# ConsenSys/wittgenstein

Hardware: NVIDIA H100
Metric: simulated-ms/sec, GSFSignature 65,536 nodes (higher is better)
Workload: dtype u64 bitmaps / int32

## Files before the change

### wittgenstein_b200/csrc/wtg_cuda.cu

```cuda
#include <cuda_runtime.h>
#include <unistd.h>

#include <cstdio>
#include <cstdlib>
#include <stdexcept>
#include <string>
#include <vector>

#include "wtg_engine.hpp"

namespace wtg {

#define CUDA_OK(x)                                                                                       \
  do {                                                                                                   \
    cudaError_t e_ = (x);                                                                                \
    if (e_ != cudaSuccess) throw std::runtime_error(std::string("CUDA: ") + cudaGetErrorString(e_) + " at " #x); \
  } while (0)

constexpr int SCAN_THREADS = 256;
constexpr int SCAN_ITEMS = 4;
constexpr int SCAN_TILE = SCAN_THREADS * SCAN_ITEMS;

__global__ void k_begin(Dev d, int mode) {
  if (threadIdx.x >= 32) return;
// ... 97 lines not shown
    for (int n = d.n0; n < d.n0 + d.nLoc; ++n) idx += (u64)hCondPick(d, n, idx, true);
  }
}
__global__ void k_hpick_publish(Dev d) {
  const int blk = blockIdx.x, nBlk = gridDim.x;
  if (!d.ctl->error)
    for (int n = d.n0 + blk * blockDim.x + threadIdx.x; n < d.n0 + d.nLoc; n += nBlk * blockDim.x) hPickPublish(d, n);
  if (blk == 0 && threadIdx.x == 0) hPickPublishHeader(d);
}
__global__ void k_hpick_xcheck(Dev d) {
  if (d.ctl->error) return;
  const int blk = blockIdx.x, nBlk = gridDim.x;
  if (blk == 0 && threadIdx.x == 0) hPickHeaders(d);
  const int upTo = hPicksBelow(d, d.rank + 1);
  for (int t = blk * blockDim.x + threadIdx.x; t < upTo; t += nBlk * blockDim.x)
    if (hPickRejects(d, t)) d.ctl->hReject = 1;
}
__global__ void k_hpick_xapply(Dev d) {
  if (d.ctl->error) return;
  const int blk = blockIdx.x, nBlk = gridDim.x;
  if (!d.ctl->hReject) {
    const u64 below = (u64)hPicksBelow(d, d.rank);
    for (int n = d.n0 + blk * blockDim.x + threadIdx.x; n < d.n0 + d.nLoc; n += nBlk * blockDim.x) hCondPick(d, n, below + (u64)d.hDrawBase[n], true);
  } else if (blk == 0 && threadIdx.x == 0) {
    hPickSerial(d);
  }
}

__global__ void k_dispatch_count(Dev d) {
  if (d.ctl->error) return;
  const int blk = blockIdx.x, nBlk = gridDim.x;
  int nEv = d.ctl->nEv;
  if (d.allCap > 0) {
    CoopWarp c;
    int gw = (blk * blockDim.x + threadIdx.x) >> 5, nw = (nBlk * blockDim.x) >> 5;
    for (int i = gw; i < nEv; i += nw) dispatchCountCoop(d, c, i);
    return;
  }
  for (int i = blk * blockDim.x + threadIdx.x; i < nEv; i += nBlk * blockDim.x) dispatchCount(d, i);
}
__global__ void k_dispatch_scatter(Dev d) {
  if (d.ctl->error) return;
  const int blk = blockIdx.x, nBlk = gridDim.x;
  int nEv = d.ctl->nEv;
  if (d.allCap > 0) {
    CoopWarp c;
    int gw = (blk * blockDim.x + threadIdx.x) >> 5, nw = (nBlk * blockDim.x) >> 5;
    for (int i = gw; i < nEv; i += nw) dispatchScatterCoop(d, c, i);
    return;
  }
  for (int i = blk * blockDim.x + threadIdx.x; i < nEv; i += nBlk * blockDim.x) dispatchScatter(d, i);
}

__global__ void __launch_bounds__(256) k_node_msgs(Dev d) {
  if (d.ctl->error) return;
  const int blk = blockIdx.x;
  int n = d.n0 + blk * blockDim.x + threadIdx.x;
  int flag = 0;
  u64 word = ~0ULL;
  if (n < d.n0 + d.nLoc && d.inboxFill[n] > 0) {
    CoopSerial cs;
    if (d.proto == PROTO_SANFERMIN || d.proto == PROTO_CAPPOS || d.proto == PROTO_SLUSH || d.proto == PROTO_SNOWFLAKE ||
        d.proto == PROTO_P2PFLOOD)
      nodeProcess(d, cs, n, 0);
    else if (d.proto == PROTO_GSF || d.proto == PROTO_PINGPONG) {
      u64 w = 0;
      int tasks = nodeProcess(d, cs, n, 1, &w);
      flag = tasks > 0 ? 1 : 0;
      if (tasks == 1) word = w;
    }
    else if (d.proto == PROTO_CASPER) {
      const u64* in = d.inbox + d.inboxOff[n];
      const Ev* bucket = d.buckets + (size_t)(d.ctl->tick & (d.ring - 1)) * (size_t)d.bcap;
      int cnt = d.inboxFill[n];
      bool simple = true;
      for (int r = 0; r < cnt && simple; ++r) {
        const Ev& ev = bucket[inboxEntry(in[r])];
        uint32_t meta = ev.kind == EV_MULTI ? d.rec[ev.aux].meta : ev.meta;
        simple = (ev.kind == EV_MSG || ev.kind == EV_MULTI) && meta == CM_ATT;
      }
      if (simple)
        nodeProcess(d, cs, n, 0);
      else
        flag = 1;
    } else
      flag = 1;
  }
  listAppend(d, flag != 0, n, d.ctl->taskCnt, d.taskList, d.taskWord, word);
}
__global__ void __launch_bounds__(256, 3) k_node_tasks(Dev d) {
  if (d.ctl->error) return;
  const int blk = blockIdx.x, nBlk = gridDim.x;
  const bool split = d.proto == PROTO_GSF || d.proto == PROTO_PINGPONG;
  const int stripe = blk & (ARENA_STRIPES - 1);
  const int cnt = d.ctl->taskCnt[stripe];
  const int sub = (blk >> 6) * 8 + (threadIdx.x >> 5);
  const int nsub = (nBlk >> 6) * 8;
  const int* list = d.taskList + (size_t)stripe * d.listStripeCap;
  const u64* words = d.taskWord + (size_t)stripe * d.listStripeCap;
  CoopWarp c;
  for (int t = sub; t < cnt; t += nsub) {
    const int n = list[t];
    const u64 w = words[t];
    if (split && w != ~0ULL)
      nodeSingleTask(d, c, n, w);
    else
      nodeProcess(d, c, n, split ? 2 : 0);
  }
}
__global__ void k_casper_fixups(Dev d) {
  const int blk = blockIdx.x;
  if (d.ctl->error || blk != 0 || threadIdx.x >= 32) return;
  CoopWarp c;
  if (d.cRandomTies && d.ctl->tieCnt > 0) casperResolveTies(d, c);
  if (d.G == 1 && d.cg->createdThisTick > 1) casperRenumber(d, c);
}
__device__ __forceinline__ Pair pairAdd(Pair x, Pair y) {
  Pair r;
  r.a = x.a + y.a;
  r.b = x.b + y.b;
  return r;
}
__device__ __forceinline__ Pair blockExclusive(Pair v, Pair& total) {
  __shared__ Pair warpSums[33];
  int lane = threadIdx.x & 31, warp = threadIdx.x >> 5, nw = blockDim.x >> 5;
  Pair inc = v;
#pragma unroll
  for (int o = 1; o < 32; o <<= 1) {
    int ta = __shfl_up_sync(0xffffffffu, inc.a, o), tb = __shfl_up_sync(0xffffffffu, inc.b, o);
    if (lane >= o) {
      inc.a += ta;
      inc.b += tb;
    }
  }
  __syncthreads();
  if (lane == 31) warpSums[warp] = inc;
  __syncthreads();
  if (warp == 0) {
    Pair w;
    w.a = lane < nw ? warpSums[lane].a : 0;
    w.b = lane < nw ? warpSums[lane].b : 0;
    Pair wi = w;
#pragma unroll
    for (int o = 1; o < 32; o <<= 1) {
      int ta = __shfl_up_sync(0xffffffffu, wi.a, o), tb = __shfl_up_sync(0xffffffffu, wi.b, o);
      if (lane >= o) {
        wi.a += ta;
        wi.b += tb;
      }
    }
    Pair ex;
    ex.a = wi.a - w.a;
    ex.b = wi.b - w.b;
    warpSums[lane] = ex;
    if (lane == 31) warpSums[32] = wi;
  }
  __syncthreads();
  total = warpSums[32];
  Pair base = warpSums[warp];
  Pair r;
// ... 292 lines not shown
        if (d.G > 1) d.newTarget[g] = -1;
      }
      __syncwarp();
    }
    __syncthreads();
  }
}

__global__ void k_free(Dev d) {
  if (d.ctl->error) return;
  const int blk = blockIdx.x, nBlk = gridDim.x;
  const int per = d.freeCap / ARENA_STRIPES;
  const int stripe = blk & (ARENA_STRIPES - 1);
  int cnt = d.ctl->freeCnt[stripe];
  if (cnt > per) cnt = per;
  const int sub = (blk >> 6) * blockDim.x + threadIdx.x;
  const int nsub = (nBlk >> 6) * blockDim.x;
  for (int j = sub; j < cnt; j += nsub) freeApply(d, stripe * per + j);
}

__global__ void k_gsf_init_nodes(Dev d) {
  int n = d.n0 + blockIdx.x * blockDim.x + threadIdx.x;
  if (n < d.n0 + d.nLoc) gsfInitNodeBody(d, n);
}
__global__ void k_rng_candidates(Dev d, u64 s0, u64 count, u64 chunk, int maxBound, u64* out, int* outCount, int cap) {
  u64 t = (u64)blockIdx.x * blockDim.x + threadIdx.x;
  u64 start = t * chunk;
  if (start >= count) return;
  u64 len = start + chunk <= count ? chunk : count - start;
  rngCandidateChunk(d, s0, start, len, maxBound, out, outCount, cap);
}
template <class PeerT>
__global__ void k_gsf_shuffle(Dev d, int l, u64 s0, const int* liveRank, const u64* rejOrd, int nRej) {
  int n = d.n0 + blockIdx.x * blockDim.x + threadIdx.x;
  if (n < d.n0 + d.nLoc) gsfShuffleLevel<PeerT>(d, n, l, s0, liveRank, rejOrd, nRej);
}

class CudaBackend : public Backend {
 public:
  cudaStream_t st = nullptr;
  cudaStream_t side = nullptr;
  cudaEvent_t forkEv = nullptr, joinEv = nullptr;
  int devId = 0;
  void bind() const { cudaSetDevice(devId); }
  int sms = 132;
  int smemOptin = 0;
  cudaGraphExec_t tickGraph = nullptr;
  const void* graphFor = nullptr;
  bool useGraph = true;
  long long launches = 0;
  long long graphKernels = 0;
  cudaEvent_t tm0 = nullptr, tm1 = nullptr;
  enum ProfSlot { P_BEGIN, P_COND_SCAN, P_DISPATCH_COUNT, P_SCAN_PARTIAL, P_EXCHANGE, P_SCAN_FINAL, P_DISPATCH_SCATTER, P_NODE,
                  P_EMIT, P_MS_COUNT, P_MS_SCAN, P_MS_SCATTER, P_FREE, P_END, P_COND_SCORE, P_COND_SELECT, P_EMIT_PEERS, NK };
  bool profiling = false;
  std::vector<cudaEvent_t> evPool;
  std::vector<int> evKernel;
  size_t evUsed = 0;
  double profMs[NK] = {};
  long long profCnt[NK] = {};
  const char* profNames[NK] = {"k_begin", "k_cond_scan", "k_dispatch_count", "k_scan_partial", "k_exchange", "k_scan_final",
                               "k_dispatch_scatter", "k_node", "k_emit", "k_ms_count", "k_ms_scan", "k_ms_scatter", "k_free",
                               "k_end", "k_cond_score", "k_cond_select", "k_emit_peers"};

  explicit CudaBackend(int requested = -1) {
    int dev = 0;
    const char* e = std::getenv("LOCAL_RANK");
    int cnt = 0;
    CUDA_OK(cudaGetDeviceCount(&cnt));
    if (cnt == 0) throw std::runtime_error("no CUDA device");
    if (e) dev = std::atoi(e) % cnt;
    const char* e2 = std::getenv("WTG_DEVICE");
    if (e2) dev = std::atoi(e2) % cnt;
    if (requested >= 0) {
      if (requested >= cnt) throw std::invalid_argument("CUDA device " + std::to_string(requested) + " does not exist");
      dev = requested;
    }
    CUDA_OK(cudaSetDevice(dev));
    devId = dev;
    cudaDeviceProp p;
    CUDA_OK(cudaGetDeviceProperties(&p, dev));
    sms = p.multiProcessorCount;
    CUDA_OK(cudaStreamCreateWithFlags(&st, cudaStreamNonBlocking));
    CUDA_OK(cudaStreamCreateWithFlags(&side, cudaStreamNonBlocking));
    CUDA_OK(cudaEventCreateWithFlags(&forkEv, cudaEventDisableTiming));
    CUDA_OK(cudaEventCreateWithFlags(&joinEv, cudaEventDisableTiming));
    CUDA_OK(cudaDeviceGetAttribute(&smemOptin, cudaDevAttrMaxSharedMemoryPerBlockOptin, dev));
    CUDA_OK(cudaFuncSetAttribute(k_ms_count, cudaFuncAttributeMaxDynamicSharedMemorySize, smemOptin));
    CUDA_OK(cudaFuncSetAttribute(k_ms_scatter, cudaFuncAttributeMaxDynamicSharedMemorySize, smemOptin));
    const char* g = std::getenv("WTG_NO_GRAPH");
    if (g && g[0] == '1') useGraph = false;
  }
  ~CudaBackend() override {
    for (void* q : ipcOpened) cudaIpcCloseMemHandle(q);
    if (tickGraph) cudaGraphExecDestroy(tickGraph);
    if (forkEv) cudaEventDestroy(forkEv);
    if (joinEv) cudaEventDestroy(joinEv);
    if (side) cudaStreamDestroy(side);
    if (st) cudaStreamDestroy(st);
  }
  void* alloc(size_t bytes) override {
    bind();
    void* p = nullptr;
    cudaError_t e = cudaMalloc(&p, bytes);
    if (e != cudaSuccess) throw std::runtime_error("cudaMalloc of " + std::to_string(bytes) + " bytes failed: " + cudaGetErrorString(e));
    CUDA_OK(cudaMemsetAsync(p, 0, bytes, st));
    return p;
  }
  void release(void* p) override { cudaFree(p); }
  int deviceId() const override { return devId; }
  void exportShared(void* p, unsigned char* handle) override {
    bind();
    std::memset(handle, 0, 128);
    cudaIpcMemHandle_t ih;
    CUDA_OK(cudaIpcGetMemHandle(&ih, p));
    static_assert(sizeof(ih) == 64, "cudaIpcMemHandle_t");
// ... 11 lines not shown
    int dev;
    std::memcpy(&pid, handle + 64, 8);
    std::memcpy(&p, handle + 72, sizeof(p));
    std::memcpy(&dev, handle + 80, 4);
    if (pid == (long long)getpid()) {
      if (dev != devId) {
        int can = 0;
        CUDA_OK(cudaDeviceCanAccessPeer(&can, devId, dev));
        if (!can) throw std::runtime_error("GPU " + std::to_string(devId) + " cannot access GPU " + std::to_string(dev) + " (peer access)");
        cudaError_t e = cudaDeviceEnablePeerAccess(dev, 0);
        if (e != cudaSuccess && e != cudaErrorPeerAccessAlreadyEnabled) CUDA_OK(e);
        cudaGetLastError();
      }
      return p;
    }
    cudaIpcMemHandle_t ih;
    std::memcpy(&ih, handle, 64);
    void* q = nullptr;
    CUDA_OK(cudaIpcOpenMemHandle(&q, ih, cudaIpcMemLazyEnablePeerAccess));
    ipcOpened.push_back(q);
    return q;
  }
  void upload(void* dst, const void* src, size_t bytes) override {
    bind();
    CUDA_OK(cudaMemcpyAsync(dst, src, bytes, cudaMemcpyHostToDevice, st));
    CUDA_OK(cudaStreamSynchronize(st));
  }
  void download(void* dst, const void* src, size_t bytes) override {
    bind();
    CUDA_OK(cudaMemcpyAsync(dst, src, bytes, cudaMemcpyDeviceToHost, st));
    CUDA_OK(cudaStreamSynchronize(st));
  }
  void sync() override {
    bind();
    CUDA_OK(cudaStreamSynchronize(st));
    drainProfile();
  }
  void timerStart() override {
    bind();
    if (!tm0) {
      CUDA_OK(cudaEventCreate(&tm0));
      CUDA_OK(cudaEventCreate(&tm1));
    }
    CUDA_OK(cudaEventRecord(tm0, st));
  }
  double timerStopMs() override {
    bind();
    CUDA_OK(cudaEventRecord(tm1, st));
    CUDA_OK(cudaEventSynchronize(tm1));
    float ms = 0;
    CUDA_OK(cudaEventElapsedTime(&ms, tm0, tm1));
    return (double)ms;
  }
  void profileEnable(bool on) override {
    sync();
    profiling = on;
    if (on) {
      for (int i = 0; i < NK; ++i) {
        profMs[i] = 0;
        profCnt[i] = 0;
      }
    }
  }
  int profileRead(double* ms, long long* cnt, const char** names, int cap) override {
    sync();
    int k = 0;
    for (int i = 0; i < NK && k < cap; ++i, ++k) {
      ms[k] = profMs[i];
      cnt[k] = profCnt[i];
      names[k] = profNames[i];
    }
    return k;
  }
  void drainProfile() {
    for (size_t i = 0; i < evUsed; ++i) {
      float ms = 0;
      cudaEventElapsedTime(&ms, evPool[2 * i], evPool[2 * i + 1]);
      profMs[evKernel[i]] += ms;
      profCnt[evKernel[i]] += 1;
    }
    evUsed = 0;
  }
  void profBegin(int kid) {
    if (!profiling) return;
    if (evUsed * 2 + 2 > evPool.size()) {
      if (evUsed >= 8192) {
        CUDA_OK(cudaStreamSynchronize(st));
        drainProfile();
      } else {
        cudaEvent_t a, b;
        CUDA_OK(cudaEventCreate(&a));
        CUDA_OK(cudaEventCreate(&b));
        evPool.push_back(a);
        evPool.push_back(b);
        evKernel.push_back(0);
      }
    }
    evKernel[evUsed] = kid;
    CUDA_OK(cudaEventRecord(evPool[2 * evUsed], st));
  }
  void profEnd() {
    if (!profiling) return;
    CUDA_OK(cudaEventRecord(evPool[2 * evUsed + 1], st));
    ++evUsed;
  }

  void fork() {
    CUDA_OK(cudaEventRecord(forkEv, st));
    CUDA_OK(cudaStreamWaitEvent(side, forkEv, 0));
  }
  void join() {
    CUDA_OK(cudaEventRecord(joinEv, side));
    CUDA_OK(cudaStreamWaitEvent(st, joinEv, 0));
  }
  void enqueueTick(const Dev& d, int mode) {
    const int wide = sms * 8;
    const size_t msSmem = (size_t)d.msWarps * d.ring * sizeof(int);
    const bool branches = mode == 1 && !profiling && d.G == 1 && (d.proto == PROTO_GSF || d.proto == PROTO_HANDEL);
    cudaStream_t sd = branches ? side : st;
    if (mode != 3) {
      profBegin(P_BEGIN);
      k_begin<<<1, 32, 0, st>>>(d, mode);
      profEnd();
// ... 4 lines not shown
      profBegin(P_COND_SCAN);
      k_cond_mark<<<(d.nLoc + 255) / 256, 256, 0, st>>>(d);
      k_cond_nodes<0><<<ARENA_STRIPES * 19, 256, 0, st>>>(d);
      profEnd();
      profBegin(P_COND_SCORE);
      k_cond_score<<<ARENA_STRIPES * 19, 256, 0, st>>>(d);
      profEnd();
      profBegin(P_COND_SELECT);
      k_cond_nodes<1><<<ARENA_STRIPES * 19, 256, smem8, st>>>(d);
      profEnd();
      launches += 4;
      if (d.proto == PROTO_HANDEL) {
        Dev dd = d;
        dd.scanPartial = d.drawScanPartial;
        profBegin(P_SCAN_PARTIAL);
        k_scan_partial<<<wide, SCAN_THREADS, 0, st>>>(dd, 2);
        profEnd();
        profBegin(P_SCAN_FINAL);
        k_scan_final<<<wide, SCAN_THREADS, 0, st>>>(dd, 2);
        profEnd();
        if (d.G > 1) {
          profBegin(P_EXCHANGE);
          k_hpick_publish<<<sms, 256, 0, st>>>(d);
          k_x_sync<<<1, 32, 0, st>>>(d, 3);
          profEnd();
          profBegin(P_COND_SELECT);
          k_hpick_xcheck<<<sms, 256, 0, st>>>(d);
          k_hpick_xapply<<<sms, 256, 0, st>>>(d);
          profEnd();
          launches += 5;
        } else {
          profBegin(P_COND_SELECT);
          k_hpick_check<<<sms, 256, 0, st>>>(d);
          k_hpick_apply<<<sms, 256, 0, st>>>(d);
          profEnd();
          launches += 3;
        }
      }
    }
    if (mode != 2 && mode != 3) {
      profBegin(P_DISPATCH_COUNT);
      k_dispatch_count<<<wide, 256, 0, sd>>>(d);
      profEnd();
      profBegin(P_SCAN_PARTIAL);
      k_scan_partial<<<wide, SCAN_THREADS, 0, sd>>>(d, 0);
      profEnd();
      profBegin(P_SCAN_FINAL);
      k_scan_final<<<wide, SCAN_THREADS, 0, sd>>>(d, 0);
      profEnd();
      profBegin(P_DISPATCH_SCATTER);
      k_dispatch_scatter<<<wide, 256, 0, sd>>>(d);
      profEnd();
      if (branches) join();
      profBegin(P_NODE);
      k_node_msgs<<<(d.nLoc + 255) / 256, 256, 0, st>>>(d);
      k_node_tasks<<<ARENA_STRIPES * 19, 256, 0, st>>>(d);
      if (d.proto == PROTO_CASPER) {
        k_casper_fixups<<<1, 32, 0, st>>>(d);
        launches += 1;
      }
      profEnd();
      launches += 6;
    }
    profBegin(P_SCAN_PARTIAL);
    k_scan_partial<<<wide, SCAN_THREADS, 0, st>>>(d, 1);
    profEnd();
    profBegin(P_SCAN_FINAL);
    k_scan_final<<<wide, SCAN_THREADS, 0, st>>>(d, 1);
    profEnd();
    if (d.G > 1) {
      profBegin(P_EXCHANGE);
      k_x1_publish<<<sms * 2, 256, 0, st>>>(d);
      k_x_sync<<<1, 32, 0, st>>>(d, 0);
      k_x1_totals<<<1, 1, 0, st>>>(d);
      k_x1_offsets<<<sms * 2, 256, 0, st>>>(d);
      profEnd();
      launches += 4;
    }
    profBegin(P_EMIT);
    if (d.shufCap > 0) {
      k_shuffle_check<<<ARENA_STRIPES * 4, 256, 0, st>>>(d);
      k_shuffle_serial<<<1, 1, 0, st>>>(d);
      launches += 2;
    }
    k_emit<<<ARENA_STRIPES * 16, 256, 0, st>>>(d);
    if (d.allCap > 0) {
      if (d.G > 1)
        k_x_all_publish<<<8, 128, 0, st>>>(d);
      else
        k_emit_all<<<d.allWarps / 4, 128, 0, st>>>(d);
      launches += 1;
    }
    profEnd();
    if (d.proto == PROTO_P2PFLOOD) {
      profBegin(P_EMIT_PEERS);
      k_emit_peers<<<sms * 8, 128, 0, st>>>(d);
      profEnd();
      launches += 1;
    }
    if (d.G > 1) {
      profBegin(P_EXCHANGE);
      k_x_sync<<<1, 32, 0, st>>>(d, 1);
      k_x2_ingest<<<sms * 4, 256, 0, st>>>(d);
      launches += 2;
      if (d.allCap > 0) {
        k_x_all_build<<<d.allWarps / 4, 128, 0, st>>>(d);
        launches += 1;
      }
      profEnd();
// ... 111 lines not shown
```

### wittgenstein_b200/csrc/wtg_engine.hpp

```cpp
#pragma once
#include <chrono>
#include <cstdio>
#include <functional>
#include <thread>
#include <cstdlib>
#include <cstring>
#include <memory>
#include <string>
#include <vector>

#include "wtg_host.hpp"
#include "wtg_logic.cuh"
#include "wtg_types.h"

namespace wtg {

struct GsfParams {
  int nodeCount, threshold, pairingTime, timeoutPerLevelMs, periodDurationMs, acceleratedCallsCount, nodesDown;
};

struct SfParams {
  int nodeCount, threshold, pairingTime, signatureSize, replyTimeout, candidateCount;
};

struct HandelParams {
  int nodeCount, threshold, pairingTime, levelWaitTime, extraCycle, disseminationPeriodMs, fastPath, nodesDown, desynchronizedStart,
      byzantineSuicide, hiddenByzantine;
};

struct CapposParams {
  int nodeCount, threshold, pairingTime, signatureSize, timeout, candidateCount;
};

struct CasperParams {
  int cycleLength, randomOnTies, blockProducersCount, attestersPerRound, blockConstructionTime, attestationConstructionTime;
};

struct Tunables {
  long long bcap = 0, qcap = 0, poolSlotsPerNode = 0, descCap = 0, recCap = 0, ring = 0;
  long long casperVotes = 0;
  long long casperBlocks = 0;
  long long peerBits32 = 0;
  long long farCap = 0;
  long long stageWords = 0;
};

struct Backend {
  virtual ~Backend() {}
  virtual void* alloc(size_t bytes) = 0;
  virtual void release(void* p) = 0;
  virtual void upload(void* dst, const void* src, size_t bytes) = 0;
  virtual void download(void* dst, const void* src, size_t bytes) = 0;
  virtual void sync() = 0;
  virtual void tick(const Dev& d, int mode) = 0;
  virtual void ticks(const Dev& d, int count) {
    for (int i = 0; i < count; ++i) tick(d, 1);
  }
  virtual void timerStart() {}
  virtual double timerStopMs() { return 0.0; }
  virtual void profileEnable(bool) {}
  virtual int profileRead(double* ms, long long* launches, const char** names, int cap) { (void)ms; (void)launches; (void)names; (void)cap; return 0; }
  virtual void* allocShared(size_t bytes) { return alloc(bytes); }
  virtual void exportShared(void* p, unsigned char* handle) {
    std::memset(handle, 0, 128);
    std::memcpy(handle + 72, &p, sizeof(p));
  }
  virtual void* importShared(const unsigned char* handle) {
    void* p;
    std::memcpy(&p, handle + 72, sizeof(p));
    return p;
  }
  virtual int deviceId() const { return 0; }
  virtual void gsfInitNodes(const Dev& d) = 0;
  virtual void rngCandidates(const Dev& d, unsigned long long s0, unsigned long long count, int maxBound,
                             std::vector<unsigned long long>& out) = 0;
  virtual void gsfShufflePeers(const Dev& d, unsigned long long s0, const int* liveRank, const unsigned long long* rejOrd, int nRej) = 0;
};

class Engine {
 public:
  std::unique_ptr<Backend> be;
  HostModel hm;
  Dev d;
  Tunables tun;
  std::vector<void*> allocs;
  bool inited = false;
  int time = 0;
  int ringMask = 0;
  bool pendingAtNow = false;
  std::vector<int> partitionsInX;
  int msgDiscardTime = 0x7fffffff;
  std::string err;
  std::vector<int> liveRank;
  unsigned long long initDraws = 0;

  int shardRank = 0, shardWorld = 1;
  bool linked = false;
  void* xRegion = nullptr;
  size_t xBytes = 0;
  long long stageWordsWanted = 0;
  long long farWanted = 0;
  struct XLayout {
    size_t hdr, flags, items, newEv, newTarget, stage, rec, recDest, recArrival, beg, all, allCnt, proto, total;
  } xl{};
  size_t xProtoBytes = 0;
  int xAllCapWanted = 0;
  bool unevenShards = false;
  bool shardFarOk = false;

  explicit Engine(Backend* b) : be(b) { std::memset(&d, 0, sizeof(d)); }
  void setShard(int rank, int world) {
    requireNotInited();
    if (world < 1 || world > MAX_SHARDS || (world & (world - 1)) != 0) throw std::invalid_argument("the number of shards must be a power of two <= 8");
// ... 1756 lines not shown
```

### wittgenstein_b200/csrc/wtg_logic.cuh

```cuda
#pragma once
#include "wtg_types.h"

template <class T, class U>
static inline T wtg_host_fetch_add(T* p, U v) {
  T o = *p;
  *p = (T)(o + (T)v);
  return o;
}
template <class T>
static inline T wtg_host_fetch_max(T* p, T v) {
  T o = *p;
  if (v > o) *p = v;
  return o;
}
template <class T>
static inline T wtg_host_fetch_min(T* p, T v) {
  T o = *p;
  if (v < o) *p = v;
  return o;
}
template <class T>
static inline T wtg_host_cas(T* p, T a, T b) {
  T o = *p;
  if (o == a) *p = b;
// ... 650 lines not shown
  return st * per + i;
}

WTG_HD void gsfLevelCounters(const Dev& d, int n, int l, int& cV, int& cI, int& cU) {
  cV = d.cntVer[n * d.L + l];
  cI = d.cntIndiv[n * d.L + l];
  cU = d.cntUnion[n * d.L + l];
}


template <class C>
WTG_HD int gsfLastFinishedLevel(const Dev& d, C& c, int n) {
  uint32_t comp = 0;
  for (int k = 0; k < 32 / C::LANES; ++k) {
    const int l = k * C::LANES + c.lane();
    comp |= c.ballot(l >= 1 && l < d.L && d.cntVer[n * d.L + l] == (1 << (l - 1))) << (k * C::LANES);
  }
  return WTG_CTZ32(~(comp >> 1));
}

WTG_HD void gsfOnNewSig(const Dev& d, int n, uint32_t from, uint32_t meta, u64 pl) {
  int l = (int)metaLevel(meta);
  int len = d.qLen[n];
  QEntry* q = d.queue + (size_t)n * d.qcap;
  if (len + 2 > d.qcap) {
    setError(d, ERR_QUEUE_OVERFLOW, n);
    if (metaKind(meta) == PK_POOL) freeDeferred(d, n, l, (uint32_t)pl);
    return;
  }
  QEntry e;
  e.from = from;
  e.meta = meta;
  e.pl = pl;
  uint32_t* qs = d.qStamp + (size_t)n * d.qcap;
  qs[len] = 0;
  q[len++] = e;
  u64* rowS = d.indivSeen + (size_t)n * d.W64;
  u64 bit = 1ULL << (from & 63);
  if (!(rowS[from >> 6] & bit)) {
    rowS[from >> 6] |= bit;
    QEntry ie;
    ie.from = from;
    ie.meta = metaMake(PK_INDIV, (uint32_t)l, 0);
    ie.pl = 0;
    qs[len] = 0;
    q[len++] = ie;
  }
  d.qLen[n] = len;
  d.sigQueueSize[n] = len;
  statMax(d, n, ST_MAXQUEUE, (unsigned long long)len);
}

template <class C>
WTG_HD int gsfTakePeers(const Dev& d, C& c, int n, int l, int want, uint32_t* out) {
  int rem = d.remaining[n * d.L + l];
  int p = d.pos[n * d.L + l];
  int sz = 1 << (l - 1);
  int cnt = want < rem ? want : rem;
  for (int i = 0; i < cnt; ++i) {
    out[i] = peerAt(d, n, l, p);
    if (++p >= sz) p = 0;
  }
  c.sync();
  if (c.lane() == 0) {
    d.remaining[n * d.L + l] = rem - cnt;
    d.pos[n * d.L + l] = p;
  }
  c.sync();
  return cnt;
}

template <class C>
WTG_HD void gsfUpdate(const Dev& d, C& c, int n, uint32_t from, uint32_t meta, u64 pl, int item, int& outSlots, int& outDraws) {
  const int L = d.L;
  const int tick = d.ctl->tick;
  int l = (int)metaLevel(meta);
  int kind = (int)metaKind(meta);
  int k = (int)metaK(meta);
  int size = 1 << (l - 1);
  Blk b = levelBlock((int)from, l);
  u64* rowV = d.verified + (size_t)n * d.W64;
  u64* rowI = d.indivVer + (size_t)n * d.W64;
  int cV, cI, cU;
  gsfLevelCounters(d, n, l, cV, cI, cU);
  int total = d.totalCard[n];
  int cSig = kind == PK_INDIV ? 1 : kind == PK_FULL ? (1 << k) : kind == PK_INLINE ? WTG_POPC64(pl) : (int)(pl >> 32);
  if (c.lane() == 0) {
    statAdd(d, n, ST_UPDATES, 1ULL);
    WTG_ATOMIC_ADD(&d.lvVer[n * L + l], 1u);
  }

  if (cSig == 1) {
    u64 bit = 1ULL << (from & 63);
    u64 wI = rowI[from >> 6], wV = rowV[from >> 6];
    c.sync();
    if (!(wI & bit)) {
      if (c.lane() == 0) rowI[from >> 6] = wI | bit;
      cI += 1;
      if (!(wV & bit)) cU += 1;
    }
    c.sync();
  }

  bool changed = false;
  bool superset = (kind == PK_FULL && k >= l);
  if (superset) {
    bool resetRemaining = false;
    for (int i = 1; i < L && i <= k; ++i) {
      int ci = d.cntVer[n * L + i];
      int si = 1 << (i - 1);
      if (ci != si) {
        Blk wb = levelBlock(n ^ (1 << (i - 1)), i);
        for (int w = c.lane(); w < wb.nw; w += C::LANES) rowV[wb.w0 + w] |= wb.mask;
        total += si - ci;
        if (c.lane() == 0) {
          d.cntVer[n * L + i] = si;
          d.cntUnion[n * L + i] = si;
          d.lvVer[n * L + i] += 1;
        }
// ... 46 lines not shown
        }
      } else if (kind == PK_INLINE) {
        if (c.lane() == 0) {
          u64 cur = rowV[b.w0];
          u64 nv = pl | (rowI[b.w0] & b.mask) | (merge ? (cur & b.mask) : 0ULL);
          rowV[b.w0] = (cur & ~b.mask) | nv;
        }
      } else {
        const u64* sig = d.pool[l] + (size_t)(uint32_t)pl * (size_t)b.nw;
        for (int w = c.lane(); w < b.nw; w += C::LANES) {
          u64 nv = sig[w] | rowI[b.w0 + w];
          if (merge) nv |= rowV[b.w0 + w];
          rowV[b.w0 + w] = nv;
        }
      }
      total += cM - cV;
      cV = cM;
      cU = cM;
      if (c.lane() == 0) d.cntVer[n * L + l] = cV;
      c.sync();
    }
  }
  if (c.lane() == 0) {
    d.cntIndiv[n * L + l] = cI;
    d.cntUnion[n * L + l] = cU;
    d.totalCard[n] = total;
  }
  if (kind == PK_POOL && c.lane() == 0) {
    freeDeferred(d, n, l, (uint32_t)pl);
    statAdd(d, n, ST_UPDATEWORDS, (unsigned long long)((changed ? 4 : 3) * b.nw));
  }
  c.sync();

  outSlots = 0;
  outDraws = 0;
  if (!changed) return;

  for (int i = l + c.lane(); i < L; i += C::LANES) d.remaining[n * L + i] = 1 << (i - 1);
  c.sync();

  if (d.accel > 0) {
    int kf = gsfLastFinishedLevel(d, c, n);
    int nSend = 0;
    for (int cur = l; cur <= kf && cur < L - 1;) {
      ++cur;
      if (d.remaining[n * L + cur] > 0) ++nSend;
    }
    if (nSend > 0) {
      int base = descAlloc(d, c, n, nSend);
      int sub = 0;
      long long sentMsgs = 0, sentBytes = 0;
      for (int cur = l; cur <= kf && cur < L - 1;) {
        ++cur;
        uint32_t dests[MAX_ACC];
        int cnt = gsfTakePeers(d, c, n, cur, d.accel, dests);
        if (cnt == 0) continue;
        sentMsgs += cnt;
        sentBytes += (long long)cnt * msgSize(cur);
        if (base >= 0 && c.lane() == 0) {
          Desc ds;
          ds.item = (uint32_t)(d.nLoc + item);
          ds.sub = (uint32_t)sub;
          ds.from = (uint32_t)n;
          ds.evKind = EV_MSG;
          ds.meta = metaMake(PK_FULL, (uint32_t)cur, (uint32_t)kf);
          ds.pl = 0;
          ds.target = 0;
          ds.aux = 0;
          if (cnt == 1) {
            ds.dkind = DK_SEND_SINGLE;
            ds.to = dests[0];
            ds.nDest = 1;
          } else {
            int off = destAlloc(d, n, cnt);
            if (off >= 0)
              for (int i = 0; i < cnt; ++i) d.destScratch[off + i] = dests[i];
            ds.dkind = DK_SEND_MULTI;
            ds.to = (uint32_t)(off < 0 ? 0 : off);
            ds.nDest = (uint32_t)(off < 0 ? 0 : cnt);
          }
          d.desc[base + sub] = ds;
        }
        ++sub;
      }
      if (c.lane() == 0) {
        d.msgSent[n] += sentMsgs;
        d.bytesSent[n] += sentBytes;
        statAdd(d, n, ST_MULTISENDS, (unsigned long long)sub);
      }
      outSlots = sub;
      outDraws = sub;
    }
  }
  if (c.lane() == 0 && d.doneAt[n] == 0 && total >= d.threshold) d.doneAt[n] = tick;
  c.sync();
}

template <class C>
WTG_HD void gsfDoCycle(const Dev& d, C& c, int n, int item, int& outSlots, int& outDraws) {
  constexpr int K = 32 / C::LANES;
  const int L = d.L;
  const int tick = d.ctl->tick;
  const u64* rowV = d.verified + (size_t)n * d.W64;
  const int kf = gsfLastFinishedLevel(d, c, n);
  uint32_t sendMask = 0;
  int carry = 0;
  for (int k = 0; k < K; ++k) {
    const int l = k * C::LANES + c.lane();
    const bool valid = l >= 1 && l < L;
    const int cv = l < L ? d.cntVer[n * L + l] : 0;
    const int rem = valid ? d.remaining[n * L + l] : 0;
    int total;
    const int prefix = carry + c.exclusiveScan(cv, total);
    carry += total;
    const int size = valid ? (1 << (l - 1)) : 0;
    const int card = (kf >= l - 1) ? (1 << kf) : prefix;
    const bool started = tick >= l * d.timeoutPerLevel || card >= size;
    sendMask |= c.ballot(valid && rem > 0 && started) << (k * C::LANES);
  }
  const int nSend = WTG_POPC32(sendMask);
  const int base = descAlloc(d, c, n, nSend + 1);
  unsigned long long words = 0;
  int bytes = 0;
  carry = 0;
  for (int k = 0; k < K; ++k) {
    const int l = k * C::LANES + c.lane();
    const bool snd = (sendMask >> l) & 1u;
    const int size = l >= 1 && l < L ? (1 << (l - 1)) : 0;
    int total;
// ... 268 lines not shown
    ds.from = (uint32_t)n;
    ds.evKind = EV_MSG;
    ds.meta = em.sendMeta;
    ds.pl = em.sendPl;
    ds.target = 0;
    ds.aux = 0;
    if (em.nSend == 1) {
      ds.dkind = DK_SEND_SINGLE;
      ds.to = em.dst[0];
      ds.nDest = 1;
    } else {
      int off = destAlloc(d, n, 2 * em.nSend);
      if (off >= 0)
        for (int i = 0; i < em.nSend; ++i) d.destScratch[off + i] = em.dst[i];
      ds.dkind = DK_SEND_MULTI;
      ds.to = (uint32_t)(off < 0 ? 0 : off);
      ds.nDest = off < 0 ? 0u : (uint32_t)em.nSend;
      ds.aux = DESC_SHUFFLEK;
    }
    d.desc[base + sub] = ds;
    ++sub;
    d.msgSent[n] += em.nSend;
    d.bytesSent[n] += (long long)em.nSend * msgBytes;
  }
  if (em.task) {
    Desc ds;
    ds.dkind = DK_INSERT_AT;
    ds.item = (uint32_t)(d.nLoc + item);
    ds.sub = (uint32_t)sub;
    ds.from = (uint32_t)n;
    ds.to = (uint32_t)n;
    ds.nDest = 0;
    ds.evKind = EV_TASK;
    ds.meta = em.taskMeta;
    ds.pl = em.taskPl;
    ds.target = em.taskAt;
    ds.aux = 0;
    d.desc[base + sub] = ds;
  }
}

WTG_HD u64 inboxMake(int item, int entry) { return ((u64)(uint32_t)item << 32) | (u64)(uint32_t)entry; }
WTG_HD int inboxItem(u64 w) { return (int)(w >> 32); }
WTG_HD int inboxEntry(u64 w) { return (int)(w & 0xFFFFFFFFULL); }

}
#include "wtg_handel.cuh"
#include "wtg_casper.cuh"
#include "wtg_cappos.cuh"
#include "wtg_avalanche.cuh"
#include "wtg_p2p.cuh"
namespace wtg {

template <class C>
WTG_HD void deliver(const Dev& d, C& c, int n, const Ev& ev, uint32_t from, uint32_t meta, u64 pl, int item) {
  int slots = 0, draws = 0;
  bool isTask = (ev.kind == EV_TASK || ev.kind == EV_PERIODIC);
  uint32_t envFrom = isTask ? (uint32_t)n : from;
  bool ok = !d.ndown[n] && d.npart[envFrom] == d.npart[n];
  if (!ok) {
    if (d.proto == PROTO_GSF && (ev.kind == EV_MSG || ev.kind == EV_TASK) && metaKind(meta) == PK_POOL && c.lane() == 0)
      freeDeferred(d, n, (int)metaLevel(meta), (uint32_t)pl);
    if (d.proto == PROTO_HANDEL && (ev.kind == EV_MSG || ev.kind == EV_TASK) && metaKind(meta) == PK_POOL && c.lane() == 0)
      hRelease(d, n, (int)metaLevel(meta), (uint32_t)pl, false);
  } else if (d.proto == PROTO_HANDEL) {
    if (ev.kind == EV_MSG || ev.kind == EV_MULTI) {
      if (c.lane() == 0) {
        d.msgReceived[n] += 1;
        d.bytesReceived[n] += hMsgSize((int)metaLevel(meta));
        statAdd(d, n, ST_DELIVERIES, 1ULL);
        hOnNewSig(d, n, from, meta, pl);
      }
      c.sync();
    } else if (ev.kind == EV_TASK) {
      if (c.lane() == 0) statAdd(d, n, ST_TASKS, 1ULL);
      hUpdate(d, c, n, from, meta, pl, ev.aux, item, slots, draws);
    } else {
      if (c.lane() == 0) statAdd(d, n, ST_TASKS, 1ULL);
      hDissemination(d, c, n, item, slots, draws);
    }
  } else if (d.proto == PROTO_GSF) {
    if (ev.kind == EV_MSG || ev.kind == EV_MULTI) {
      if (c.lane() == 0) {
        d.msgReceived[n] += 1;
        d.bytesReceived[n] += msgSize((int)metaLevel(meta));
        statAdd(d, n, ST_DELIVERIES, 1ULL);
        gsfOnNewSig(d, n, from, meta, pl);
      }
      c.sync();
    } else if (ev.kind == EV_TASK) {
      if (c.lane() == 0) statAdd(d, n, ST_TASKS, 1ULL);
      gsfUpdate(d, c, n, from, meta, pl, item, slots, draws);
    } else {
      if (c.lane() == 0) statAdd(d, n, ST_TASKS, 1ULL);
      gsfDoCycle(d, c, n, item, slots, draws);
    }
  } else if (d.proto == PROTO_CASPER) {
    casperDeliver(d, c, n, ev.kind, meta, pl, item, slots, draws);
  } else if (d.proto == PROTO_CAPPOS) {
    if (c.lane() == 0) cpHandle(d, n, from, meta, pl, item, slots, draws);
    slots = c.bcast(slots, 0);
    draws = c.bcast(draws, 0);
  } else if (d.proto == PROTO_SANFERMIN) {
    if (c.lane() == 0) sfHandle(d, n, from, meta, pl, item, slots, draws);
    slots = c.bcast(slots, 0);
    draws = c.bcast(draws, 0);
  } else if (d.proto == PROTO_SLUSH || d.proto == PROTO_SNOWFLAKE) {
    if (c.lane() == 0) avHandle(d, n, from, meta, pl, item, slots, draws);
    slots = c.bcast(slots, 0);
    draws = c.bcast(draws, 0);
  } else if (d.proto == PROTO_P2PFLOOD) {
    if (c.lane() == 0) floodHandle(d, n, from, pl, item, slots, draws);
    slots = c.bcast(slots, 0);
    draws = c.bcast(draws, 0);
  } else if (d.proto == PROTO_PINGPONG) {
    if (c.lane() == 0) {
      d.msgReceived[n] += 1;
      d.bytesReceived[n] += 1;
      statAdd(d, n, ST_DELIVERIES, 1ULL);
    }
    if (meta == PP_PING) {
      int base = descAlloc(d, c, n, 1);
      if (c.lane() == 0) {
        if (base >= 0) {
          Desc ds;
          ds.dkind = DK_SEND_SINGLE;
          ds.item = (uint32_t)(d.nLoc + item);
          ds.sub = 0;
          ds.from = (uint32_t)n;
          ds.to = from;
          ds.nDest = 1;
          ds.evKind = EV_MSG;
          ds.meta = PP_PONG;
          ds.pl = 0;
          ds.target = 0;
          ds.aux = 0;
          d.desc[base] = ds;
        }
        d.msgSent[n] += 1;
        d.bytesSent[n] += 1;
      }
      slots = 1;
      draws = 1;
    } else {
      if (c.lane() == 0) d.pong[n] += 1;
    }
    c.sync();
  }
  if (c.lane() == 0) {
    d.evSlots[item] = slots;
    d.evDraws[item] = draws;
  }
}


template <class C>
WTG_HD int nodeProcess(const Dev& d, C& c, int n, int filter, u64* skippedWord = nullptr) {
  int cnt = d.inboxFill[n];
  if (cnt == 0) return 0;
  const u64* in = d.inbox + d.inboxOff[n];
  const Ev* bucket = d.buckets + (size_t)(d.ctl->tick & (d.ring - 1)) * (size_t)d.bcap;
  int lastItem = -1;
  int skipped = 0;
  for (int r = 0; r < cnt; ++r) {
    int bestItem = 0x7fffffff;
    u64 bestW = 0;
    for (int i = c.lane(); i < cnt; i += C::LANES) {
      u64 w = in[i];
      int it = inboxItem(w);
      if (it > lastItem && it < bestItem) {
        bestItem = it;
        bestW = w;
      }
    }
    int mn = c.minv(bestItem);
    uint32_t who = c.ballot(bestItem == mn);
    int src = c.first(who);
    u64 w = c.bcast64(bestW, src);
    lastItem = mn;
    int item = inboxItem(w), entry = inboxEntry(w);
    Ev ev = bucket[entry];
    bool isTask = ev.kind == EV_TASK || ev.kind == EV_PERIODIC;
    if ((filter == 1 && isTask) || (filter == 2 && !isTask)) {
      ++skipped;
      if (skippedWord) *skippedWord = w;
      continue;
    }
    uint32_t from = ev.from, meta = ev.meta;
    u64 pl = ev.pl;
    if (ev.kind == EV_MULTI) {
      const MultiRec& rc = d.rec[ev.aux];
      from = rc.from;
      meta = rc.meta;
      pl = rc.pl;
    }
    deliver(d, c, n, ev, from, meta, pl, item);
  }
  if (c.lane() == 0) {
    if (filter != 2) statMax(d, n, ST_MAXINBOX, (unsigned long long)cnt);
    if (filter == 0 || filter == 2 || skipped == 0) d.inboxFill[n] = 0;
  }
  return skipped;
}
template <class C>
WTG_HD void nodeSingleTask(const Dev& d, C& c, int n, u64 w) {
  const Ev* bucket = d.buckets + (size_t)(d.ctl->tick & (d.ring - 1)) * (size_t)d.bcap;
  Ev ev = bucket[inboxEntry(w)];
  deliver(d, c, n, ev, ev.from, ev.meta, ev.pl, inboxItem(w));
  if (c.lane() == 0) d.inboxFill[n] = 0;
}

WTG_HD void dispatchCount(const Dev& d, int i) {
  const Ctl& ctl = *d.ctl;
  int p = ctl.nEv - 1 - i;
  const Ev& ev = d.buckets[(size_t)(ctl.tick & (d.ring - 1)) * (size_t)d.bcap + i];
  int m = 1, rep = 0;
  if (ev.kind == EV_MULTI) {
    const MultiRec& rc = d.rec[ev.aux];
    int j = (int)rc.cur;
    m = 0;
    int lastOwner = d.rank;
    while (j < (int)rc.n && d.recArrival[rc.off + j] == ctl.tick) {
      const int to = (int)d.recDest[rc.off + j];
      lastOwner = ownerOf(d, to);
      if (lastOwner == d.rank) {
        WTG_ATOMIC_ADD(&d.inboxCnt[to], 1);
        ++m;
      }
      ++j;
    }
    rep = (j < (int)rc.n && lastOwner == d.rank) ? 1 : 0;
  } else {
    WTG_ATOMIC_ADD(&d.inboxCnt[ev.to], 1);
  }
  d.subCount[p] = m + rep;
}

WTG_HD void dispatchScatter(const Dev& d, int i) {
  const Ctl& ctl = *d.ctl;
  int p = ctl.nEv - 1 - i;
  const size_t be = (size_t)(ctl.tick & (d.ring - 1)) * (size_t)d.bcap + i;
  const Ev& ev = d.buckets[be];
  int item0 = d.itemBase[p];
  const u64 bkey = d.G > 1 ? d.bucketKey[be] : 0;
  if (ev.kind == EV_MULTI) {
    MultiRec& rc = d.rec[ev.aux];
    int j = (int)rc.cur, m = 0;
    int lastOwner = d.rank;
    while (j < (int)rc.n && d.recArrival[rc.off + j] == ctl.tick) {
      int to = (int)d.recDest[rc.off + j];
      lastOwner = ownerOf(d, to);
      if (lastOwner == d.rank) {
        int s = d.inboxOff[to] + WTG_ATOMIC_ADD(&d.inboxFill[to], 1);
        d.inbox[s] = inboxMake(item0 + m, i);
        if (d.G > 1) d.itemKey[item0 + m] = bkey | keySub(j);
        ++m;
      }
      ++j;
    }
    if (j < (int)rc.n && lastOwner == d.rank) {
      int dst_ = i & (ARENA_STRIPES - 1), dper_ = d.descCap / ARENA_STRIPES;
      int di = WTG_ATOMIC_ADD(&d.ctl->descCnt[dst_], 1);
// ... 613 lines not shown
```

### wittgenstein_b200/network.py

```python
import ctypes as C
import threading

import numpy as np

from . import _lib
from ._lib import WtgError


def _p(a, t):
    return a.ctypes.data_as(C.POINTER(t))


_tls = threading.local()


def set_thread_device(device):
    _tls.device = device


class Network:
    def __init__(self, _api=None, device=None, shard=None):
        self.api = _api or _lib.api()
        if device is None:
            device = getattr(_tls, "device", None)
# ... 87 lines not shown
        return self.api.check(self.api.msgs_size(self.h))

    def msgs_size_at(self, t):
        return self.api.check(self.api.msgs_size_at(self.h, int(t)))

    def peek_messages(self, cap=1 << 16):
        a = [np.zeros(cap, np.int32) for _ in range(6)]
        total = self.api.check(self.api.peek_messages(self.h, *[_p(x, C.c_int) for x in a], int(cap)))
        k = min(total, cap)
        return total, dict(zip(["from", "to", "sent_at", "arriving_at", "kind", "msg_type"], [x[:k] for x in a]))

    def stop_node(self, node_id):
        self.api.check(self.api.stop_node(self.h, int(node_id)))

    def start_node(self, node_id):
        self.api.check(self.api.start_node(self.h, int(node_id)))

    def partition(self, part):
        self.api.check(self.api.partition(self.h, float(part)))

    def end_partition(self):
        self.api.check(self.api.end_partition(self.h))

    def rng_state(self):
        return int(self.api.rng_state(self.h))

    def counters(self):
        out = np.zeros((5, self.local_count), np.int64)
        self.api.check(self.api.node_counters(self.h, _p(out, C.c_longlong)))
        return out

    def attrs(self):
        n = self.node_count
        x = np.zeros(n, np.int32); y = np.zeros(n, np.int32); e = np.zeros(n, np.int32); c = np.zeros(n, np.int32)
        s = np.zeros(n, np.float64); d = np.zeros(n, np.uint8)
        self.api.check(self.api.node_attrs(self.h, _p(x, C.c_int), _p(y, C.c_int), _p(e, C.c_int), _p(c, C.c_int),
                                           _p(s, C.c_double), _p(d, C.c_ubyte)))
        return dict(x=x, y=y, extra=e, city=c, speed=s, down=d)

    def stats(self):
        out = np.zeros(26, np.int64)
        self.api.check(self.api.stats(self.h, _p(out, C.c_longlong)))
        keys = ["deliveries", "tasks", "cond_runs", "draws", "eval_entries", "eval_words", "updates", "cycles", "sends",
                "multi_sends", "send_words", "events", "max_queue", "max_bucket", "max_inbox", "rec_top", "rec_dest_top",
                "kernel_launches", "min_pool_free", "init_draws", "ring", "bcap", "qcap", "peer_bits", "update_words", "reevaluated"]
        return dict(zip(keys, out.tolist()))

    def timer_start(self):
        self.api.check(self.api.timer_start(self.h))

    def timer_stop_ms(self):
        return float(self.api.timer_stop_ms(self.h))

    def profile_enable(self, on=True):
        self.api.check(self.api.profile_enable(self.h, 1 if on else 0))

    def profile_read(self):
        cap = 64
        ms = (C.c_double * cap)()
        cnt = (C.c_longlong * cap)()
        names = (C.c_char_p * cap)()
        k = self.api.check(self.api.profile_read(self.h, ms, cnt, names, cap))
        return {names[i].decode(): (ms[i], cnt[i]) for i in range(k)}
```

Measured before the change: 5018.

## Specialize node kernels for GSF at compile time and cut register pressure

```diff
diff --git a/wittgenstein_b200/csrc/wtg_cuda.cu b/wittgenstein_b200/csrc/wtg_cuda.cu
--- a/wittgenstein_b200/csrc/wtg_cuda.cu
+++ b/wittgenstein_b200/csrc/wtg_cuda.cu
@@ -173,24 +173,26 @@
   for (int i = blk * blockDim.x + threadIdx.x; i < nEv; i += nBlk * blockDim.x) dispatchScatter(d, i);
 }
 
+template <int P>
 __global__ void __launch_bounds__(256) k_node_msgs(Dev d) {
   if (d.ctl->error) return;
+  const int proto = protoOf<P>(d);
   const int blk = blockIdx.x;
   int n = d.n0 + blk * blockDim.x + threadIdx.x;
   int flag = 0;
   u64 word = ~0ULL;
   if (n < d.n0 + d.nLoc && d.inboxFill[n] > 0) {
     CoopSerial cs;
-    if (d.proto == PROTO_SANFERMIN || d.proto == PROTO_CAPPOS || d.proto == PROTO_SLUSH || d.proto == PROTO_SNOWFLAKE ||
-        d.proto == PROTO_P2PFLOOD)
-      nodeProcess(d, cs, n, 0);
-    else if (d.proto == PROTO_GSF || d.proto == PROTO_PINGPONG) {
+    if (proto == PROTO_SANFERMIN || proto == PROTO_CAPPOS || proto == PROTO_SLUSH || proto == PROTO_SNOWFLAKE ||
+        proto == PROTO_P2PFLOOD)
+      nodeProcess<P>(d, cs, n, 0);
+    else if (proto == PROTO_GSF || proto == PROTO_PINGPONG) {
       u64 w = 0;
-      int tasks = nodeProcess(d, cs, n, 1, &w);
+      int tasks = nodeProcess<P>(d, cs, n, 1, &w);
       flag = tasks > 0 ? 1 : 0;
       if (tasks == 1) word = w;
     }
-    else if (d.proto == PROTO_CASPER) {
+    else if (proto == PROTO_CASPER) {
       const u64* in = d.inbox + d.inboxOff[n];
       const Ev* bucket = d.buckets + (size_t)(d.ctl->tick & (d.ring - 1)) * (size_t)d.bcap;
       int cnt = d.inboxFill[n];
@@ -201,7 +203,7 @@
         simple = (ev.kind == EV_MSG || ev.kind == EV_MULTI) && meta == CM_ATT;
       }
       if (simple)
-        nodeProcess(d, cs, n, 0);
+        nodeProcess<P>(d, cs, n, 0);
       else
         flag = 1;
     } else
@@ -209,10 +211,14 @@
   }
   listAppend(d, flag != 0, n, d.ctl->taskCnt, d.taskList, d.taskWord, word);
 }
-__global__ void __launch_bounds__(256, 3) k_node_tasks(Dev d) {
-  if (d.ctl->error) return;
-  const int blk = blockIdx.x, nBlk = gridDim.x;
-  const bool split = d.proto == PROTO_GSF || d.proto == PROTO_PINGPONG;
+template <int P>
+constexpr int nodeTaskBlocks() { return P == PROTO_GSF ? 4 : 3; }
+template <int P>
+__global__ void __launch_bounds__(256, nodeTaskBlocks<P>()) k_node_tasks(Dev d) {
+  if (d.ctl->error) return;
+  const int proto = protoOf<P>(d);
+  const int blk = blockIdx.x, nBlk = gridDim.x;
+  const bool split = proto == PROTO_GSF || proto == PROTO_PINGPONG;
   const int stripe = blk & (ARENA_STRIPES - 1);
   const int cnt = d.ctl->taskCnt[stripe];
   const int sub = (blk >> 6) * 8 + (threadIdx.x >> 5);
@@ -223,10 +229,10 @@
   for (int t = sub; t < cnt; t += nsub) {
     const int n = list[t];
     const u64 w = words[t];
-    if (split && w != ~0ULL)
-      nodeSingleTask(d, c, n, w);
+    if (P == PROTO_GSF || (split && w != ~0ULL))
+      nodeProcess<P>(d, c, n, 2, nullptr, w);
     else
-      nodeProcess(d, c, n, split ? 2 : 0);
+      nodeProcess<P>(d, c, n, split ? 2 : 0);
   }
 }
 __global__ void k_casper_fixups(Dev d) {
@@ -625,8 +631,9 @@
   long long graphKernels = 0;
   cudaEvent_t tm0 = nullptr, tm1 = nullptr;
   enum ProfSlot { P_BEGIN, P_COND_SCAN, P_DISPATCH_COUNT, P_SCAN_PARTIAL, P_EXCHANGE, P_SCAN_FINAL, P_DISPATCH_SCATTER, P_NODE,
-                  P_EMIT, P_MS_COUNT, P_MS_SCAN, P_MS_SCATTER, P_FREE, P_END, P_COND_SCORE, P_COND_SELECT, P_EMIT_PEERS, NK };
-  bool profiling = false;
+                  P_EMIT, P_MS_COUNT, P_MS_SCAN, P_MS_SCATTER, P_FREE, P_END, P_COND_SCORE, P_COND_SELECT, P_EMIT_PEERS,
+                  P_NODE_MSGS, P_NODE_TASKS, NK };
+  int profiling = 0;
   std::vector<cudaEvent_t> evPool;
   std::vector<int> evKernel;
   size_t evUsed = 0;
@@ -634,7 +641,7 @@
   long long profCnt[NK] = {};
   const char* profNames[NK] = {"k_begin", "k_cond_scan", "k_dispatch_count", "k_scan_partial", "k_exchange", "k_scan_final",
                                "k_dispatch_scatter", "k_node", "k_emit", "k_ms_count", "k_ms_scan", "k_ms_scatter", "k_free",
-                               "k_end", "k_cond_score", "k_cond_select", "k_emit_peers"};
+                               "k_end", "k_cond_score", "k_cond_select", "k_emit_peers", "k_node_msgs", "k_node_tasks"};
 
   explicit CudaBackend(int requested = -1) {
     int dev = 0;
@@ -752,7 +759,7 @@
     CUDA_OK(cudaEventElapsedTime(&ms, tm0, tm1));
     return (double)ms;
   }
-  void profileEnable(bool on) override {
+  void profileEnable(int on) override {
     sync();
     profiling = on;
     if (on) {
@@ -765,10 +772,11 @@
   int profileRead(double* ms, long long* cnt, const char** names, int cap) override {
     sync();
     int k = 0;
-    for (int i = 0; i < NK && k < cap; ++i, ++k) {
+    for (int i = 0; i < NK && k < cap; ++i) {
+      if ((i == P_NODE_MSGS || i == P_NODE_TASKS) && !profCnt[i]) continue;
       ms[k] = profMs[i];
       cnt[k] = profCnt[i];
-      names[k] = profNames[i];
+      names[k++] = profNames[i];
     }
     return k;
   }
@@ -879,9 +887,15 @@
       k_dispatch_scatter<<<wide, 256, 0, sd>>>(d);
       profEnd();
       if (branches) join();
-      profBegin(P_NODE);
-      k_node_msgs<<<(d.nLoc + 255) / 256, 256, 0, st>>>(d);
-      k_node_tasks<<<ARENA_STRIPES * 19, 256, 0, st>>>(d);
+      const bool gsf = d.proto == PROTO_GSF;
+      const bool byKernel = profiling == 2;
+      profBegin(byKernel ? P_NODE_MSGS : P_NODE);
+      (gsf ? k_node_msgs<PROTO_GSF> : k_node_msgs<PROTO_ANY>)<<<(d.nLoc + 255) / 256, 256, 0, st>>>(d);
+      if (byKernel) {
+        profEnd();
+        profBegin(P_NODE_TASKS);
+      }
+      (gsf ? k_node_tasks<PROTO_GSF> : k_node_tasks<PROTO_ANY>)<<<ARENA_STRIPES * 19, 256, 0, st>>>(d);
       if (d.proto == PROTO_CASPER) {
         k_casper_fixups<<<1, 32, 0, st>>>(d);
         launches += 1;
diff --git a/wittgenstein_b200/csrc/wtg_engine.hpp b/wittgenstein_b200/csrc/wtg_engine.hpp
--- a/wittgenstein_b200/csrc/wtg_engine.hpp
+++ b/wittgenstein_b200/csrc/wtg_engine.hpp
@@ -58,7 +58,7 @@
   }
   virtual void timerStart() {}
   virtual double timerStopMs() { return 0.0; }
-  virtual void profileEnable(bool) {}
+  virtual void profileEnable(int) {}
   virtual int profileRead(double* ms, long long* launches, const char** names, int cap) { (void)ms; (void)launches; (void)names; (void)cap; return 0; }
   virtual void* allocShared(size_t bytes) { return alloc(bytes); }
   virtual void exportShared(void* p, unsigned char* handle) {
diff --git a/wittgenstein_b200/csrc/wtg_logic.cuh b/wittgenstein_b200/csrc/wtg_logic.cuh
--- a/wittgenstein_b200/csrc/wtg_logic.cuh
+++ b/wittgenstein_b200/csrc/wtg_logic.cuh
@@ -726,19 +726,16 @@
 }
 
 template <class C>
-WTG_HD int gsfTakePeers(const Dev& d, C& c, int n, int l, int want, uint32_t* out) {
+WTG_HD int gsfTakePeers(const Dev& d, C& c, int n, int l, int want, int& first) {
   int rem = d.remaining[n * d.L + l];
   int p = d.pos[n * d.L + l];
   int sz = 1 << (l - 1);
   int cnt = want < rem ? want : rem;
-  for (int i = 0; i < cnt; ++i) {
-    out[i] = peerAt(d, n, l, p);
-    if (++p >= sz) p = 0;
-  }
+  first = p;
   c.sync();
   if (c.lane() == 0) {
     d.remaining[n * d.L + l] = rem - cnt;
-    d.pos[n * d.L + l] = p;
+    d.pos[n * d.L + l] = (p + cnt) & (sz - 1);
   }
   c.sync();
   return cnt;
@@ -891,8 +888,9 @@
       long long sentMsgs = 0, sentBytes = 0;
       for (int cur = l; cur <= kf && cur < L - 1;) {
         ++cur;
-        uint32_t dests[MAX_ACC];
-        int cnt = gsfTakePeers(d, c, n, cur, d.accel, dests);
+        int first;
+        int cnt = gsfTakePeers(d, c, n, cur, d.accel, first);
+        const int wrap = (1 << (cur - 1)) - 1;
         if (cnt == 0) continue;
         sentMsgs += cnt;
         sentBytes += (long long)cnt * msgSize(cur);
@@ -908,12 +906,12 @@
           ds.aux = 0;
           if (cnt == 1) {
             ds.dkind = DK_SEND_SINGLE;
-            ds.to = dests[0];
+            ds.to = peerAt(d, n, cur, first);
             ds.nDest = 1;
           } else {
             int off = destAlloc(d, n, cnt);
             if (off >= 0)
-              for (int i = 0; i < cnt; ++i) d.destScratch[off + i] = dests[i];
+              for (int i = 0; i < cnt; ++i) d.destScratch[off + i] = peerAt(d, n, cur, (first + i) & wrap);
             ds.dkind = DK_SEND_MULTI;
             ds.to = (uint32_t)(off < 0 ? 0 : off);
             ds.nDest = (uint32_t)(off < 0 ? 0 : cnt);
@@ -1288,18 +1286,22 @@
 #include "wtg_p2p.cuh"
 namespace wtg {
 
-template <class C>
+constexpr int PROTO_ANY = -1;
+template <int P>
+WTG_HD int protoOf(const Dev& d) { return P == PROTO_ANY ? d.proto : P; }
+template <int P, class C>
 WTG_HD void deliver(const Dev& d, C& c, int n, const Ev& ev, uint32_t from, uint32_t meta, u64 pl, int item) {
+  const int proto = protoOf<P>(d);
   int slots = 0, draws = 0;
   bool isTask = (ev.kind == EV_TASK || ev.kind == EV_PERIODIC);
   uint32_t envFrom = isTask ? (uint32_t)n : from;
   bool ok = !d.ndown[n] && d.npart[envFrom] == d.npart[n];
   if (!ok) {
-    if (d.proto == PROTO_GSF && (ev.kind == EV_MSG || ev.kind == EV_TASK) && metaKind(meta) == PK_POOL && c.lane() == 0)
+    if (proto == PROTO_GSF && (ev.kind == EV_MSG || ev.kind == EV_TASK) && metaKind(meta) == PK_POOL && c.lane() == 0)
       freeDeferred(d, n, (int)metaLevel(meta), (uint32_t)pl);
-    if (d.proto == PROTO_HANDEL && (ev.kind == EV_MSG || ev.kind == EV_TASK) && metaKind(meta) == PK_POOL && c.lane() == 0)
+    if (proto == PROTO_HANDEL && (ev.kind == EV_MSG || ev.kind == EV_TASK) && metaKind(meta) == PK_POOL && c.lane() == 0)
       hRelease(d, n, (int)metaLevel(meta), (uint32_t)pl, false);
-  } else if (d.proto == PROTO_HANDEL) {
+  } else if (proto == PROTO_HANDEL) {
     if (ev.kind == EV_MSG || ev.kind == EV_MULTI) {
       if (c.lane() == 0) {
         d.msgReceived[n] += 1;
@@ -1315,8 +1317,8 @@
       if (c.lane() == 0) statAdd(d, n, ST_TASKS, 1ULL);
       hDissemination(d, c, n, item, slots, draws);
     }
-  } else if (d.proto == PROTO_GSF) {
-    if (ev.kind == EV_MSG || ev.kind == EV_MULTI) {
+  } else if (proto == PROTO_GSF) {
+    if (!isTask) {
       if (c.lane() == 0) {
         d.msgReceived[n] += 1;
         d.bytesReceived[n] += msgSize((int)metaLevel(meta));
@@ -1331,25 +1333,25 @@
       if (c.lane() == 0) statAdd(d, n, ST_TASKS, 1ULL);
       gsfDoCycle(d, c, n, item, slots, draws);
     }
-  } else if (d.proto == PROTO_CASPER) {
+  } else if (proto == PROTO_CASPER) {
     casperDeliver(d, c, n, ev.kind, meta, pl, item, slots, draws);
-  } else if (d.proto == PROTO_CAPPOS) {
+  } else if (proto == PROTO_CAPPOS) {
     if (c.lane() == 0) cpHandle(d, n, from, meta, pl, item, slots, draws);
     slots = c.bcast(slots, 0);
     draws = c.bcast(draws, 0);
-  } else if (d.proto == PROTO_SANFERMIN) {
+  } else if (proto == PROTO_SANFERMIN) {
     if (c.lane() == 0) sfHandle(d, n, from, meta, pl, item, slots, draws);
     slots = c.bcast(slots, 0);
     draws = c.bcast(draws, 0);
-  } else if (d.proto == PROTO_SLUSH || d.proto == PROTO_SNOWFLAKE) {
+  } else if (proto == PROTO_SLUSH || proto == PROTO_SNOWFLAKE) {
     if (c.lane() == 0) avHandle(d, n, from, meta, pl, item, slots, draws);
     slots = c.bcast(slots, 0);
     draws = c.bcast(draws, 0);
-  } else if (d.proto == PROTO_P2PFLOOD) {
+  } else if (proto == PROTO_P2PFLOOD) {
     if (c.lane() == 0) floodHandle(d, n, from, pl, item, slots, draws);
     slots = c.bcast(slots, 0);
     draws = c.bcast(draws, 0);
-  } else if (d.proto == PROTO_PINGPONG) {
+  } else if (proto == PROTO_PINGPONG) {
     if (c.lane() == 0) {
       d.msgReceived[n] += 1;
       d.bytesReceived[n] += 1;
@@ -1390,30 +1392,34 @@
 }
 
 
-template <class C>
-WTG_HD int nodeProcess(const Dev& d, C& c, int n, int filter, u64* skippedWord = nullptr) {
-  int cnt = d.inboxFill[n];
+template <int P = PROTO_ANY, class C>
+WTG_HD int nodeProcess(const Dev& d, C& c, int n, int filter, u64* skippedWord = nullptr, u64 only = ~0ULL) {
+  const bool known = only != ~0ULL;
+  int cnt = known ? 1 : d.inboxFill[n];
   if (cnt == 0) return 0;
   const u64* in = d.inbox + d.inboxOff[n];
   const Ev* bucket = d.buckets + (size_t)(d.ctl->tick & (d.ring - 1)) * (size_t)d.bcap;
   int lastItem = -1;
   int skipped = 0;
   for (int r = 0; r < cnt; ++r) {
-    int bestItem = 0x7fffffff;
-    u64 bestW = 0;
-    for (int i = c.lane(); i < cnt; i += C::LANES) {
-      u64 w = in[i];
-      int it = inboxItem(w);
-      if (it > lastItem && it < bestItem) {
-        bestItem = it;
-        bestW = w;
-      }
-    }
-    int mn = c.minv(bestItem);
-    uint32_t who = c.ballot(bestItem == mn);
-    int src = c.first(who);
-    u64 w = c.bcast64(bestW, src);
-    lastItem = mn;
+    u64 w = only;
+    if (!known) {
+      int bestItem = 0x7fffffff;
+      u64 bestW = 0;
+      for (int i = c.lane(); i < cnt; i += C::LANES) {
+        u64 x = in[i];
+        int it = inboxItem(x);
+        if (it > lastItem && it < bestItem) {
+          bestItem = it;
+          bestW = x;
+        }
+      }
+      int mn = c.minv(bestItem);
+      uint32_t who = c.ballot(bestItem == mn);
+      int src = c.first(who);
+      w = c.bcast64(bestW, src);
+      lastItem = mn;
+    }
     int item = inboxItem(w), entry = inboxEntry(w);
     Ev ev = bucket[entry];
     bool isTask = ev.kind == EV_TASK || ev.kind == EV_PERIODIC;
@@ -1430,20 +1436,13 @@
       meta = rc.meta;
       pl = rc.pl;
     }
-    deliver(d, c, n, ev, from, meta, pl, item);
+    deliver<P>(d, c, n, ev, from, meta, pl, item);
   }
   if (c.lane() == 0) {
     if (filter != 2) statMax(d, n, ST_MAXINBOX, (unsigned long long)cnt);
     if (filter == 0 || filter == 2 || skipped == 0) d.inboxFill[n] = 0;
   }
   return skipped;
-}
-template <class C>
-WTG_HD void nodeSingleTask(const Dev& d, C& c, int n, u64 w) {
-  const Ev* bucket = d.buckets + (size_t)(d.ctl->tick & (d.ring - 1)) * (size_t)d.bcap;
-  Ev ev = bucket[inboxEntry(w)];
-  deliver(d, c, n, ev, ev.from, ev.meta, ev.pl, inboxItem(w));
-  if (c.lane() == 0) d.inboxFill[n] = 0;
 }
 
 WTG_HD void dispatchCount(const Dev& d, int i) {
diff --git a/wittgenstein_b200/network.py b/wittgenstein_b200/network.py
--- a/wittgenstein_b200/network.py
+++ b/wittgenstein_b200/network.py
@@ -163,8 +163,8 @@
     def timer_stop_ms(self):
         return float(self.api.timer_stop_ms(self.h))
 
-    def profile_enable(self, on=True):
-        self.api.check(self.api.profile_enable(self.h, 1 if on else 0))
+    def profile_enable(self, on=True, handlers=False):
+        self.api.check(self.api.profile_enable(self.h, (2 if handlers else 1) if on else 0))
 
     def profile_read(self):
         cap = 64
```

New measurement: 5091, median of 6. No clear change (+1.5%).
